# sumitsk/algp

Hardware: AMD Instinct MI355X
Metric: GP-fit+MI-score throughput (N train x M candidates) (higher is better)
Workload: dtype f64

## Files before the change

algp_amd/csrc/gemm.hip:

```cpp
#include "common.h"
#include <hip/hip_ext.h>
#include "mfma.h"
#include "gemm_sched.h"
#include <algorithm>
#include <type_traits>
#include <stdio.h>
#include <stdlib.h>

namespace algp {

template <typename T>
struct GemmArgs {
    const T* A;
    const T* B;
    const T* C;
    T* D;
    int64_t lda, ldb, ldc, ldd;
    int64_t sA, sB, sC, sD;
    int tiles_m, tiles_n, ktiles;
    T alpha, beta;
    int lower_only;
    int ktri;
    int kcut;
    const T* stat_w;
    T* stat_out;
    int64_t stat_ld;
    Sched sch;
    T* part;
};

template <typename T, int DP_, int FAM_ = 0>
struct GenGemmArgs : GemmArgs<T> {
    static constexpr int DP = DP_;
    static constexpr int FAM = FAM_;
    const T* rx;
    const T* cx;
    const int* rk;
    int64_t col0;
    int64_t ncols;
    int kernel;
    T os;
};
template <typename A>
struct gen_dp { static constexpr int value = 0; };
template <typename T, int DP, int FAM>
struct gen_dp<GenGemmArgs<T, DP, FAM>> { static constexpr int value = DP; };

typedef __attribute__((address_space(3))) void* lds_vp;
typedef const __attribute__((address_space(1))) void* glb_vp;

template <int CTRL>
__device__ __forceinline__ float dpp_row(float x) {
    return __int_as_float(__builtin_amdgcn_update_dpp(0, __float_as_int(x), CTRL, 0xf, 0xf, false));
}
template <int CTRL>
__device__ __forceinline__ double dpp_row(double x) {
    const int lo = __builtin_amdgcn_update_dpp(0, __double2loint(x), CTRL, 0xf, 0xf, false);
    const int hi = __builtin_amdgcn_update_dpp(0, __double2hiint(x), CTRL, 0xf, 0xf, false);
    return __hiloint2double(hi, lo);
}
template <typename T>
__device__ __forceinline__ T row16_sum(T x) {
    x += dpp_row<0x128>(x);
    x += dpp_row<0x124>(x);
    x += dpp_row<0x122>(x);
    x += dpp_row<0x121>(x);
    return x;
}

template <typename T>
struct VrGemmArgs : GemmArgs<T> {
    const int64_t* cidx;
    const int* ckind;
    int64_t M;
    union {
        int64_t ncol0;
        const int64_t* cpool;
    };
    const T* Xs;
    const T* Cp;
    int64_t n_pool;
    int DP, kernel;
    T os, noise;
    const T* tw;
};

template <typename T>
struct VrWGemmArgs : VrGemmArgs<T> {};
template <typename T>
struct VrxGemmArgs : VrGemmArgs<T> {};
template <typename T>
struct VrxWGemmArgs : VrxGemmArgs<T> {};

template <typename T>
__device__ __forceinline__ T vr_pool_cov(const VrGemmArgs<T>& g, int64_t prow, int64_t pcol, const T (&xrow)[MAXD], const T* xcol) {
    if (g.Cp) return g.Cp[prow * g.n_pool + pcol];
    T r2 = (T)0;
#pragma unroll
    for (int d = 0; d < MAXD; ++d) {
        const T df = xrow[d] - xcol[d];
        r2 += df * df;
    }
    T cv;
    if (g.kernel == ALGP_KERNEL_RBF) cv = g.os * kexp((T)-0.5 * r2);
    else if (g.kernel == ALGP_KERNEL_MATERN15) {
        const T rr = sqrt(r2) * (T)1.7320508075688772;
        cv = g.os * ((T)1 + rr) * kexp(-rr);
    } else cv = kval<T, 1>(g.kernel, g.os, r2);
    if (prow == pcol) cv += g.noise;
    return cv;
}

template <typename T, bool WEIGHTED, bool RECT, typename ACC>
__device__ __forceinline__ void vr_epilogue(const VrGemmArgs<T>& g, char* smem, const ACC (&acc)[4][4], int64_t m0, int64_t n0, int bn,
                                            int wr, int wc, int lane, int tid, const int64_t* cpool = nullptr) {
    using F = MF<T>;
    const int fr = lane & 15;
    T* red = reinterpret_cast<T*>(smem);
    T* xr = reinterpret_cast<T*>(smem + 2048);
    T* xc = reinterpret_cast<T*>(smem + 2048 + 8192);
    int64_t* pr = reinterpret_cast<int64_t*>(smem + 2048 + 16384);
    int64_t* pc = pr + 128;
    int* kr = reinterpret_cast<int*>(pc + 128);
    int* mc = kr + 128;
    T* wcol = reinterpret_cast<T*>(kr + 128);
    __syncthreads();
    {
        const int t = tid & 127;
        const bool is_col = tid >= 128;
        int64_t p;
        int ordinary;
        if (RECT && is_col) {
            const int64_t hp = cpool[n0 + t];
            ordinary = hp >= 0 ? 1 : 0;
            p = ordinary ? hp : 0;
        } else {
            const int64_t gi = (!RECT && is_col) ? g.ncol0 + n0 + t : m0 + t;
            const bool valid = gi < g.M;
            p = valid ? g.cidx[gi] : 0;
            ordinary = (valid && g.ckind[gi] < 0) ? 1 : 0;
        }
        (is_col ? pc : pr)[t] = p;
        if constexpr (WEIGHTED) {
            if (is_col) wcol[t] = ordinary ? g.tw[p] : (T)0;
            else kr[t] = ordinary;
        } else {
            (is_col ? mc : kr)[t] = ordinary;
        }
        if (!g.Cp) {
            T* x = (is_col ? xc : xr) + t * MAXD;
#pragma unroll
            for (int d = 0; d < MAXD; ++d) x[d] = d < g.DP ? g.Xs[p * g.DP + d] : (T)0;
        }
    }
    __syncthreads();
#pragma unroll
    for (int i = 0; i < 4; ++i)
#pragma unroll
        for (int r = 0; r < 4; ++r) {
            const int row = wr * 64 + i * 16 + F::row_of(lane, r);
            const int64_t prow = pr[row];
            const T kap = kr[row] ? (T)1 : (T)0;
            T xrow[MAXD];
#pragma unroll
            for (int d = 0; d < MAXD; ++d) xrow[d] = xr[row * MAXD + d];
            T s2 = (T)0;
            if constexpr (WEIGHTED) {
                T es[4], we[4];
#pragma unroll
                for (int j = 0; j < 4; ++j) {
                    const int col = wc * 64 + j * 16 + fr;
                    const int64_t pcol = pc[col];
                    const T cv = vr_pool_cov<T>(g, prow, pcol, xrow, xc + col * MAXD);
                    const T wgt = wcol[col];
                    const T e = kap * cv - acc[i][j][r];
                    es[j] = wgt != (T)0 ? e : (T)0;
                    we[j] = wgt * es[j];
                }
                s2 = kfma(we[0], es[0], we[1] * es[1]);
                s2 = kfma(we[2], es[2], s2);
                s2 = kfma(we[3], es[3], s2);
            } else {
#pragma unroll
                for (int j = 0; j < 4; ++j) {
                    const int col = wc * 64 + j * 16 + fr;
                    const int64_t pcol = pc[col];
                    const T cv = vr_pool_cov<T>(g, prow, pcol, xrow, xc + col * MAXD);
                    T e = kap * cv - acc[i][j][r];
                    e = mc[col] ? e : (T)0;
                    s2 += e * e;
                }
            }
            s2 = row16_sum<T>(s2);
            if (fr == 0) red[wc * 128 + row] = s2;
        }
    __syncthreads();
    if (tid < 128) g.stat_out[(int64_t)bn * g.stat_ld + m0 + tid] = red[tid] + red[128 + tid];
}

template <typename T>
struct PvrGemmArgs : VrGemmArgs<T> {
    const int64_t* uidx;
    int64_t U;
    T* E;
    int64_t lde;
};

template <typename T, typename ACC>
__device__ __forceinline__ void pvr_epilogue(const PvrGemmArgs<T>& g, char* smem, const ACC (&acc)[4][4], int64_t m0, int64_t n0, int wr,
                                             int wc, int lane, int tid) {
    using F = MF<T>;
    const int fr = lane & 15;
    T* xr = reinterpret_cast<T*>(smem);
    T* xc = reinterpret_cast<T*>(smem + 8192);
    int64_t* pr = reinterpret_cast<int64_t*>(smem + 16384);
    int64_t* pc = pr + 128;
    int* kr = reinterpret_cast<int*>(pc + 128);
    T* wcol = reinterpret_cast<T*>(kr + 128);
    __syncthreads();
    {
        const int t = tid & 127;
        const bool is_col = tid >= 128;
        const int64_t gi = is_col ? g.ncol0 + n0 + t : m0 + t;
        const bool valid = is_col ? gi < g.M : gi < g.U;
        const int64_t p = valid ? (is_col ? g.cidx[gi] : g.uidx[gi]) : 0;
        (is_col ? pc : pr)[t] = p;
        if (is_col) wcol[t] = (valid && g.ckind[gi] < 0) ? (g.tw ? sqrt(g.tw[p]) : (T)1) : (T)0;
        else kr[t] = valid ? 1 : 0;
        if (!g.Cp) {
            T* x = (is_col ? xc : xr) + t * MAXD;
#pragma unroll
            for (int d = 0; d < MAXD; ++d) x[d] = d < g.DP ? g.Xs[p * g.DP + d] : (T)0;
        }
    }
    __syncthreads();
#pragma unroll
    for (int i = 0; i < 4; ++i)
#pragma unroll
        for (int r = 0; r < 4; ++r) {
            const int row = wr * 64 + i * 16 + F::row_of(lane, r);
            const int64_t prow = pr[row];
            const bool rowon = kr[row] != 0;
            T xrow[MAXD];
#pragma unroll
            for (int d = 0; d < MAXD; ++d) xrow[d] = xr[row * MAXD + d];
            T* Er = g.E + (m0 + row) * g.lde + n0;
#pragma unroll
            for (int j = 0; j < 4; ++j) {
                const int col = wc * 64 + j * 16 + fr;
                const int64_t pcol = pc[col];
                const T cv = vr_pool_cov<T>(g, prow, pcol, xrow, xc + col * MAXD);
                const T sw = wcol[col];
                Er[col] = (rowon && sw != (T)0) ? sw * (cv - acc[i][j][r]) : (T)0;
            }
        }
}

#ifndef ALGP_GEMM_XOR_MASK
#define ALGP_GEMM_XOR_MASK 2
#endif
template <typename T, bool STATS = false, typename Args = GemmArgs<T>, bool SCHED = false>
__global__ __launch_bounds__(256, 2) void gemm_nt_kernel_dma4(Args g) {
    constexpr int GDP = gen_dp<Args>::value;
    constexpr bool GEN = GDP > 0;
    constexpr bool VR = std::is_base_of<VrGemmArgs<T>, Args>::value;
    static_assert(!(VR && STATS), "one epilogue per kernel");
    static_assert(!(VR && SCHED), "the scheduled form serves the sweep's products only");
    static_assert(!GEN || (SCHED && !STATS), "generated C tiles: the scheduled update product only");
    constexpr int NST = 4;
    using F = MF<T>;
    using acc_t = typename F::acc_t;
    using chunk_t = typename F::chunk_t;
    constexpr int EPC = F::EPC;
    constexpr int BK = 4 * EPC;

    constexpr int GEN_LDS = GEN ? 2 * 128 * GDP * (int)sizeof(T) + 128 * (int)sizeof(int) : 0;
    __shared__ __attribute__((aligned(1024))) char smem[NST * 16384 + (SCHED && STATS ? 4096 : 0) + GEN_LDS];

    const int nwg = gridDim.x;
    int bm, bn;
    int kskip = 0;
    int nkt;
    int slice = -1, nunits = 1, ui = 0;
    if constexpr (SCHED) {
        nunits = sched_count<!GEN>(g.sch, blockIdx.x);
        const SchedUnit u = sched_unit<!GEN>(g.sch, blockIdx.x, 0);
        bm = u.tile / g.tiles_n;
        bn = u.tile - bm * g.tiles_n;
        kskip = u.kb0 * (128 / BK);
        nkt = (u.kb1 - u.kb0) * (128 / BK);
        slice = u.slice;
    } else {
    if (g.ktri) {
        int local = blockIdx.x >> 3;
        bm = blockIdx.x & 7;
        while (bm < g.tiles_m && local > bm) { local -= bm + 1; bm += 8; }
        if (bm >= g.tiles_m) return;
        bn = local;
    } else {
        int sid;
        {
            const int id = blockIdx.x, xcd = id & 7, q = nwg >> 3, r = nwg & 7;
            sid = (xcd < r ? xcd * (q + 1) : r * (q + 1) + (xcd - r) * q) + (id >> 3);
        }
        if (g.lower_only) {
            bm = (int)((sqrt(8.0 * (double)sid + 1.0) - 1.0) * 0.5);
            while ((int64_t)(bm + 1) * (bm + 2) / 2 <= sid) ++bm;
            while ((int64_t)bm * (bm + 1) / 2 > sid) --bm;
            bn = sid - (int)((int64_t)bm * (bm + 1) / 2);
        } else {
            bm = sid / g.tiles_n;
            bn = sid - bm * g.tiles_n;
        }
    }
    kskip = g.ktri ? bm * (128 / BK) : 0;
    nkt = g.ktiles * 2 - kskip;
    if (g.kcut && (bn + 1) * (128 / BK) < nkt) nkt = (bn + 1) * (128 / BK);
    }
    const int tid = threadIdx.x, lane = tid & 63;
    const int wave = __builtin_amdgcn_readfirstlane(tid >> 6);
    const int wr = wave >> 1, wc = wave & 1;
    const int64_t bz = blockIdx.y;

    const int srow = lane >> 2;
    const int schunk = (lane & 3) ^ ((lane >> 4) & ALGP_GEMM_XOR_MASK);
    const T* Ag = g.A + bz * g.sA + ((int64_t)bm * 128 + 32 * wave + srow) * g.lda + schunk * EPC + (int64_t)kskip * BK;
    const T* Bg = g.B + bz * g.sB + ((int64_t)bn * 128 + 32 * wave + srow) * g.ldb + schunk * EPC + (int64_t)kskip * BK;
    auto stage = [&](int st, int kt) {
        char* As = smem + st * 16384 + wave * 2048;
        char* Bs = As + 8192;
#pragma unroll
        for (int i = 0; i < 2; ++i) {
            __builtin_amdgcn_global_load_lds((glb_vp)(Ag + (int64_t)(16 * i) * g.lda + (int64_t)kt * BK),
                                             (lds_vp)(As + i * 1024), 16, 0, 0);
            __builtin_amdgcn_global_load_lds((glb_vp)(Bg + (int64_t)(16 * i) * g.ldb + (int64_t)kt * BK),
                                             (lds_vp)(Bs + i * 1024), 16, 0, 0);
        }
    };

    const int fr = lane & 15, fg = lane >> 4;
    const int coff = ((fg ^ ((fr >> 2) & ALGP_GEMM_XOR_MASK)) << 4);
    const int aoff = (wr * 64 + fr) * 64 + coff;
    const int boff = (wc * 64 + fr) * 64 + coff;

    acc_t acc[4][4];
    typedef T gen_vec_t __attribute__((ext_vector_type(GEN ? GDP : 1)));
    gen_vec_t gx;
    int gk = -1;
    auto gen_load = [&](int ubm, int ubn) {
        if constexpr (GEN) {
            int t = tid & 127;
            asm volatile("" : "+v"(t));
            const int64_t row = (int64_t)ubm * 128 + t;
            const T* src = wave >= 2 ? g.cx + (g.col0 + (int64_t)ubn * 128 + t) * GDP : g.rx + row * GDP;
            gx = *reinterpret_cast<const gen_vec_t*>(src);
            gk = g.rk[row];
            asm volatile("" ::: "memory");
        }
    };
    gen_load(bm, bn);
#pragma unroll
    for (int t = 0; t < NST - 1; ++t)
        if (t < nkt) stage(t, t);

    auto fread = [&](int st, chunk_t (&a)[4], chunk_t (&b)[4]) {
        const char* As = smem + st * 16384;
        const char* Bs = As + 8192;
#pragma unroll
        for (int t = 0; t < 4; ++t) a[t] = *reinterpret_cast<const chunk_t*>(As + aoff + t * 1024);
#pragma unroll
        for (int t = 0; t < 4; ++t) b[t] = *reinterpret_cast<const chunk_t*>(Bs + boff + t * 1024);
    };
    auto fmac = [&](const chunk_t (&a)[4], const chunk_t (&b)[4]) {
#pragma unroll
        for (int j = 0; j < 4; ++j)
#pragma unroll
            for (int e = 0; e < EPC; ++e)
#pragma unroll
                for (int i = 0; i < 4; ++i) acc[i][j] = F::mfma(a[i][e], b[j][e], acc[i][j]);
    };
    auto arrive = [&](int younger) {
        if (younger >= 2) __builtin_amdgcn_s_waitcnt(0x0F78);
        else if (younger >= 1) __builtin_amdgcn_s_waitcnt(0x0F74);
        else __builtin_amdgcn_s_waitcnt(0x0F70);
        __builtin_amdgcn_s_barrier();
        asm volatile("" ::: "memory");
    };

    int st = 0;
    for (;;) {
#pragma unroll
    for (int i = 0; i < 4; ++i)
#pragma unroll
        for (int j = 0; j < 4; ++j)
#pragma unroll
            for (int r = 0; r < 4; ++r) acc[i][j][r] = (T)0;
    for (int kt = 0; kt < nkt; ++kt) {
        arrive(nkt - 1 - kt);
        chunk_t a[4], b[4];
        fread(st, a, b);
        if (kt + NST - 1 < nkt) stage(st == 0 ? NST - 1 : st - 1, kt + NST - 1);
        fmac(a, b);
        st = (st + 1 == NST) ? 0 : st + 1;
    }
    const int64_t m0 = (int64_t)bm * 128, n0 = (int64_t)bn * 128;
    const int cur_bn = bn, cur_slice = slice;
    if constexpr (GEN) {
        if (cur_slice < 0) {
            T* xr = reinterpret_cast<T*>(smem + NST * 16384);
            T* xc = xr + 128 * GDP;
            int* kr = reinterpret_cast<int*>(xc + 128 * GDP);
            int t = tid & 127;
            asm volatile("" : "+v"(t));
            *reinterpret_cast<gen_vec_t*>((wave >= 2 ? xc : xr) + t * GDP) = gx;
            if (wave < 2) kr[t] = gk;
        }
        asm volatile("" ::: "memory");
    }
    if constexpr (SCHED) {
        if (++ui < nunits) {
            const SchedUnit u = sched_unit<!GEN>(g.sch, blockIdx.x, ui);
            bm = u.tile / g.tiles_n;
            bn = u.tile - bm * g.tiles_n;
            nkt = (u.kb1 - u.kb0) * (128 / BK);
            slice = u.slice;
            gen_load(bm, bn);
            Ag = g.A + ((int64_t)bm * 128 + 32 * wave + srow) * g.lda + schunk * EPC + (int64_t)u.kb0 * 128;
            Bg = g.B + ((int64_t)bn * 128 + 32 * wave + srow) * g.ldb + schunk * EPC + (int64_t)u.kb0 * 128;
#pragma unroll
            for (int t = 0; t < NST - 1; ++t) stage((st + t) & (NST - 1), t);
        }
    }

    if constexpr (std::is_same<Args, PvrGemmArgs<T>>::value) {
        pvr_epilogue<T>(g, smem, acc, m0, n0, wr, wc, lane, tid);
        return;
    } else if constexpr (VR) {
        constexpr bool WEIGHTED = std::is_same<Args, VrWGemmArgs<T>>::value || std::is_same<Args, VrxWGemmArgs<T>>::value;
        if constexpr (std::is_base_of<VrxGemmArgs<T>, Args>::value)
            vr_epilogue<T, WEIGHTED, true>(g, smem, acc, m0, n0, (int)bz * g.tiles_n + cur_bn, wr, wc, lane, tid,
                                           reinterpret_cast<const int64_t*>(reinterpret_cast<const char*>(g.cpool) +
                                                                            bz * g.sB * (int64_t)sizeof(T)));
        else
            vr_epilogue<T, WEIGHTED, false>(g, smem, acc, m0, n0, cur_bn, wr, wc, lane, tid);
        return;
    }
    const T alpha = g.alpha, beta = g.beta;
    const T* Cb = g.C + bz * g.sC;
    T* Db = g.D + bz * g.sD;
    if (SCHED && !STATS && cur_slice >= 0) {
        T* P = g.part + (int64_t)cur_slice * (128 * 128);
#pragma unroll
        for (int i = 0; i < 4; ++i)
#pragma unroll
            for (int r = 0; r < 4; ++r) {
                const int row = wr * 64 + i * 16 + F::row_of(lane, r);
#pragma unroll
                for (int j = 0; j < 4; ++j) P[row * 128 + wc * 64 + j * 16 + fr] = alpha * acc[i][j][r];
            }
    } else if constexpr (GEN) {
        const T* xr = reinterpret_cast<const T*>(smem + NST * 16384);
        const T* xc = xr + 128 * GDP;
        const int* kr = reinterpret_cast<const int*>(xc + 128 * GDP);
        __builtin_amdgcn_s_waitcnt(0xC07F);
        __builtin_amdgcn_s_barrier();
        asm volatile("" ::: "memory");
        int ln = lane;
        asm volatile("" : "+v"(ln));
        const int gfr = ln & 15;
        T xcol[4][GDP];
#pragma unroll
        for (int j = 0; j < 4; ++j)
#pragma unroll
            for (int d = 0; d < GDP; ++d) xcol[j][d] = xc[(wc * 64 + j * 16 + gfr) * GDP + d];
        const int64_t gc = g.col0 + n0 + wc * 64 + gfr;
        const T os = g.os;
        const int64_t ncols = g.ncols;
        auto tile_out = [&](auto kform) {
#pragma unroll
            for (int i = 0; i < 4; ++i)
#pragma unroll
                for (int r = 0; r < 4; ++r) {
                    const int row = wr * 64 + i * 16 + F::row_of(ln, r);
                    T xrow[GDP];
#pragma unroll
                    for (int d = 0; d < GDP; ++d) xrow[d] = xr[row * GDP + d];
                    const int kind = kr[row];
                    T* Dr = Db + (m0 + row) * g.ldd + n0 + wc * 64 + gfr;
#pragma unroll
                    for (int j = 0; j < 4; ++j) {
                        const T cv = bt_entry<T, GDP>(decltype(kform)::value, os, xrow, xcol[j], kind, gc + 16 * j, ncols);
                        Dr[j * 16] = alpha * acc[i][j][r] + beta * cv;
                        if (j & 1) __builtin_amdgcn_sched_barrier(0);
                    }
                }
        };
        if constexpr (Args::FAM == 0) {
            if (g.kernel == ALGP_KERNEL_RBF) tile_out(std::integral_constant<int, ALGP_KERNEL_RBF>{});
            else tile_out(std::integral_constant<int, ALGP_KERNEL_MATERN15>{});
        } else {
            if (g.kernel == ALGP_KERNEL_MATERN05) tile_out(std::integral_constant<int, ALGP_KERNEL_MATERN05>{});
            else tile_out(std::integral_constant<int, ALGP_KERNEL_MATERN25>{});
        }
    } else if (beta != (T)0) {
#pragma unroll
        for (int i = 0; i < 4; ++i) {
            T cv[4][4];
#pragma unroll
            for (int r = 0; r < 4; ++r) {
                const int64_t gi = m0 + wr * 64 + i * 16 + F::row_of(lane, r);
#pragma unroll
                for (int j = 0; j < 4; ++j) cv[r][j] = Cb[gi * g.ldc + n0 + wc * 64 + j * 16 + fr];
            }
#pragma unroll
            for (int r = 0; r < 4; ++r) {
                const int64_t gi = m0 + wr * 64 + i * 16 + F::row_of(lane, r);
#pragma unroll
                for (int j = 0; j < 4; ++j)
                    Db[gi * g.ldd + n0 + wc * 64 + j * 16 + fr] = alpha * acc[i][j][r] + beta * cv[r][j];
            }
        }
    } else if (!STATS) {
#pragma unroll
        for (int i = 0; i < 4; ++i)
#pragma unroll
            for (int r = 0; r < 4; ++r) {
                const int64_t gi = m0 + wr * 64 + i * 16 + F::row_of(lane, r);
#pragma unroll
                for (int j = 0; j < 4; ++j) Db[gi * g.ldd + n0 + wc * 64 + j * 16 + fr] = alpha * acc[i][j][r];
            }
    } else {
        T wv[4];
#pragma unroll
        for (int j = 0; j < 4; ++j) wv[j] = g.stat_w[n0 + wc * 64 + j * 16 + fr];
        T* red = reinterpret_cast<T*>(smem + (SCHED ? NST * 16384 : 0));
        if constexpr (!SCHED) __syncthreads();
#pragma unroll
        for (int i = 0; i < 4; ++i)
#pragma unroll
            for (int r = 0; r < 4; ++r) {
                const int row = wr * 64 + i * 16 + F::row_of(lane, r);
                T s2 = (T)0, sw = (T)0;
#pragma unroll
                for (int j = 0; j < 4; ++j) {
                    const T d = alpha * acc[i][j][r];
                    Db[(m0 + row) * g.ldd + n0 + wc * 64 + j * 16 + fr] = d;
                    s2 += d * d;
                    sw += d * wv[j];
                }
                s2 = row16_sum<T>(s2);
                sw = row16_sum<T>(sw);
                if (fr == 0) {
                    red[(wc * 128 + row) * 2 + 0] = s2;
                    red[(wc * 128 + row) * 2 + 1] = sw;
                }
            }
        if constexpr (SCHED) {
            __builtin_amdgcn_s_waitcnt(0xC07F);
            __builtin_amdgcn_s_barrier();
            asm volatile("" ::: "memory");
        } else {
            __syncthreads();
        }
        const int row = tid >> 1, q = tid & 1;
        g.stat_out[(int64_t)(2 * cur_bn + q) * g.stat_ld + m0 + row] = red[row * 2 + q] + red[(128 + row) * 2 + q];
    }
    if constexpr (!SCHED) return;
    if (ui >= nunits) return;
    __builtin_amdgcn_s_waitcnt(0x0F70);
    }
}

constexpr int FIN_STRIPS = 16;
constexpr int FIN_BATCH = 8;
template <typename T>
struct Fin {
    static constexpr int EPV = 16 / (int)sizeof(T);
    static constexpr int RPW = 256 * EPV / 128;
    static constexpr int PPT = (128 / FIN_STRIPS) / RPW;
    static constexpr int RSTEP = RPW;
    typedef T V __attribute__((ext_vector_type(EPV)));
    static_assert(PPT >= 1 && PPT * RPW * FIN_STRIPS == 128, "a strip is whole passes of the workgroup");
};

template <typename T, int NB>
__device__ __forceinline__ void finish_add(const T* P, unsigned off, typename Fin<T>::V (&v)[Fin<T>::PPT]) {
#pragma clang fp contract(off)
    using F = Fin<T>;
    typename F::V p[NB][F::PPT];
#pragma unroll
    for (int b = 0; b < NB; ++b)
#pragma unroll
        for (int i = 0; i < F::PPT; ++i)
            p[b][i] = *reinterpret_cast<const typename F::V*>(P + b * (128 * 128) + (off + i * F::RSTEP * 128));
    __builtin_amdgcn_sched_barrier(0);
#pragma unroll
    for (int b = 0; b < NB; ++b)
#pragma unroll
        for (int i = 0; i < F::PPT; ++i) v[i] += p[b][i];
}

template <typename T>
__device__ __forceinline__ void finish_sum(const T* P, unsigned off, int S, typename Fin<T>::V (&v)[Fin<T>::PPT]) {
    int q = 0;
    for (; q + FIN_BATCH <= S; q += FIN_BATCH) finish_add<T, FIN_BATCH>(P + (int64_t)q * (128 * 128), off, v);
    static_assert(FIN_BATCH == 8, "the remainder below is 4 + 2 + 1");
    if ((S - q) & 4) { finish_add<T, 4>(P + (int64_t)q * (128 * 128), off, v); q += 4; }
    if ((S - q) & 2) { finish_add<T, 2>(P + (int64_t)q * (128 * 128), off, v); q += 2; }
    if ((S - q) & 1) finish_add<T, 1>(P + (int64_t)q * (128 * 128), off, v);
}

template <typename T>
__global__ __launch_bounds__(256) void gemm_finish_kernel(const T* part, int S, int tile0, int tiles_n, T beta, const T* C, int64_t ldc,
                                                          T* D, int64_t ldd) {
#pragma clang fp contract(off)
    using F = Fin<T>;
    using V = typename F::V;
    const int j = blockIdx.x / FIN_STRIPS, strip = blockIdx.x - j * FIN_STRIPS;
    const int tile = tile0 + j, bm = tile / tiles_n, bn = tile - bm * tiles_n;
    const int lrow = strip * (128 / FIN_STRIPS) + (int)threadIdx.x / (128 / F::EPV), lcol = ((int)threadIdx.x % (128 / F::EPV)) * F::EPV;
    const int64_t row = (int64_t)bm * 128 + lrow, col = (int64_t)bn * 128 + lcol;
    V v[F::PPT];
#pragma unroll
    for (int i = 0; i < F::PPT; ++i) v[i] = beta * *reinterpret_cast<const V*>(C + (row + i * F::RSTEP) * ldc + col);
    finish_sum<T>(part + (int64_t)j * S * (128 * 128), (unsigned)(lrow * 128 + lcol), S, v);
#pragma unroll
    for (int i = 0; i < F::PPT; ++i) *reinterpret_cast<V*>(D + (row + i * F::RSTEP) * ldd + col) = v[i];
}

template <typename T, int DP, int FAM>
__global__ __launch_bounds__(256) void gemm_finish_gen_kernel(const T* part, int S, int tile0, int tiles_n, T beta, const T* rx, const T* cx,
                                                              const int* rk, int64_t col0, int64_t ncols, int kernel, T os, T* D, int64_t ldd) {
#pragma clang fp contract(off)
    using F = Fin<T>;
    using V = typename F::V;
    const int j = blockIdx.x / FIN_STRIPS, strip = blockIdx.x - j * FIN_STRIPS;
    const int tile = tile0 + j, bm = tile / tiles_n, bn = tile - bm * tiles_n;
    const int lrow = strip * (128 / FIN_STRIPS) + (int)threadIdx.x / (128 / F::EPV), lcol = ((int)threadIdx.x % (128 / F::EPV)) * F::EPV;
    const int64_t row = (int64_t)bm * 128 + lrow, col = (int64_t)bn * 128 + lcol;
    T xcol[F::EPV][DP];
#pragma unroll
    for (int e = 0; e < F::EPV; ++e)
#pragma unroll
        for (int d = 0; d < DP; ++d) xcol[e][d] = cx[(col0 + col + e) * DP + d];
    T xrow[F::PPT][DP];
    int kind[F::PPT];
#pragma unroll
    for (int i = 0; i < F::PPT; ++i) {
#pragma unroll
        for (int d = 0; d < DP; ++d) xrow[i][d] = rx[(row + i * F::RSTEP) * DP + d];
        kind[i] = rk[row + i * F::RSTEP];
    }
    V v[F::PPT];
    auto c_term = [&](auto kform) {
#pragma clang fp contract(off)
#pragma unroll
        for (int i = 0; i < F::PPT; ++i) {
            V cv;
#pragma unroll
            for (int e = 0; e < F::EPV; ++e)
                cv[e] = bt_entry<T, DP>(decltype(kform)::value, os, xrow[i], xcol[e], kind[i], col0 + col + e, ncols);
            v[i] = beta * cv;
        }
    };
    if constexpr (FAM == 0) {
        if (kernel == ALGP_KERNEL_RBF) c_term(std::integral_constant<int, ALGP_KERNEL_RBF>{});
        else c_term(std::integral_constant<int, ALGP_KERNEL_MATERN15>{});
    } else {
        if (kernel == ALGP_KERNEL_MATERN05) c_term(std::integral_constant<int, ALGP_KERNEL_MATERN05>{});
        else c_term(std::integral_constant<int, ALGP_KERNEL_MATERN25>{});
    }
    finish_sum<T>(part + (int64_t)j * S * (128 * 128), (unsigned)(lrow * 128 + lcol), S, v);
#pragma unroll
    for (int i = 0; i < F::PPT; ++i) *reinterpret_cast<V*>(D + (row + i * F::RSTEP) * ldd + col) = v[i];
}

static void launch_log_line(int klass, int64_t m, int64_t n, int64_t k, int lower_only, int batch, int ktri, int es, int kcut) {
    static FILE* launch_log = getenv("ALGP_LAUNCH_LOG") ? fopen(getenv("ALGP_LAUNCH_LOG"), "w") : nullptr;
    if (!launch_log) return;
    fprintf(launch_log, "%d %lld %lld %lld %d %d %d %d %d\n", klass, (long long)m, (long long)n, (long long)k, lower_only, batch, ktri, es, kcut);
    fflush(launch_log);
}

template <typename T>
static int gemm_check(algp_ctx* c, const char* who, const GemmNt<T>& p, int64_t* tiles) {
    if (p.m % 128 || p.n % 128 || p.k % 128 || p.k <= 0 || p.A.ld % 4 || p.B.ld % 4 || p.A.stride % 4 || p.B.stride % 4)
        return fail(c, ALGP_ERR_BAD_ARG, std::string(who) + ": operands must be padded to multiples of 128");
    const int64_t tm = p.m / 128, tn = p.n / 128;
    *tiles = p.lower_only ? tm * (tm + 1) / 2 : tm * tn;
    if (*tiles > 0x7fffffff) return fail(c, ALGP_ERR_BAD_ARG, std::string(who) + ": grid too large");
    return ALGP_OK;
}

template <typename T>
static void gemm_fill(GemmArgs<T>& g, const GemmNt<T>& p) {
    const bool inplace = !p.C.p;
    g.A = p.A.p; g.B = p.B.p; g.C = inplace ? p.D.p : p.C.p; g.D = p.D.p;
    g.lda = p.A.ld; g.ldb = p.B.ld; g.ldc = inplace ? p.D.ld : p.C.ld; g.ldd = p.D.ld;
    g.sA = p.A.stride; g.sB = p.B.stride; g.sC = inplace ? p.D.stride : p.C.stride; g.sD = p.D.stride;
    g.tiles_m = (int)(p.m / 128);
    g.tiles_n = (int)(p.n / 128);
    g.ktiles = (int)(p.k / (8 * MF<T>::EPC));
    g.alpha = p.alpha; g.beta = p.beta;
    g.lower_only = p.lower_only;
    g.ktri = p.ktri;
    g.kcut = p.kcut;
    g.stat_w = p.stat_w;
    g.stat_out = p.stat_out;
    g.stat_ld = p.stat_ld;
    g.sch = Sched();
    g.part = nullptr;
}

struct Booking { double flops, bytes; };
template <typename T>
static Booking gemm_book(const GemmNt<T>& p, int64_t tiles, double tile_elems) {
    const double tm = (double)(p.m / 128), tn = (double)(p.n / 128);
    Booking b;
    b.flops = p.ktri ? 2.0 * 128.0 * 128.0 * 128.0 * tm * (tm + 1.0) * (tm + 2.0) / 6.0 * p.batch
              : p.kcut ? 2.0 * 128.0 * 128.0 * 128.0 * tm * tn * (tn + 1.0) / 2.0 * p.batch
                       : 2.0 * 128.0 * 128.0 * (double)p.k * (double)tiles * p.batch;
    b.bytes = sizeof(T) * p.batch * ((double)tiles * tile_elems + (double)p.k * 128.0 * (tm + tn));
    launch_log_line(p.klass, p.m, p.n, p.k, p.lower_only, p.batch, p.ktri, (int)sizeof(T), p.kcut);
    return b;
}

template <typename X>
struct as_is { typedef X type; };
template <typename... P>
static int dispatch(algp_ctx* c, int klass, double flops, double bytes, void (*kernel)(P...), dim3 grid, const typename as_is<P>::type&... args) {
    hipEvent_t ev_a, ev_b;
    if (prof_launch_events(c, klass, flops, bytes, &ev_a, &ev_b)) hipExtLaunchKernelGGL(kernel, grid, dim3(256), 0, c->cur, ev_a, ev_b, 0, args...);
    else hipLaunchKernelGGL(kernel, grid, dim3(256), 0, c->cur, args...);
    ALGP_HIP(hipGetLastError());
    return ALGP_OK;
}

template <typename T, typename Args, typename... Tail>
static int launch_scheduled(algp_ctx* c, const char* who, const GemmNt<T>& p, const Booking& bk, Args& g, void (*product)(Args),
                            void (*finish)(const T*, int, int, int, T, Tail...), bool c_loaded, const typename as_is<Tail>::type&... tail) {
    const int slots = 2 * c->cu_count;
    const bool split = p.beta != (T)0 && !p.stat_out && !p.kcut && c->gemm_part.p &&
                       c->gemm_part.cap >= sizeof(T) * 128 * 128 * (size_t)slots;
    g.sch = sched_make(slots, g.tiles_m, g.tiles_n, (int)(p.k / 128), p.kcut, split ? 1 : 0);
    g.part = (T*)c->gemm_part.p;
    if (g.sch.S >= 2 && (g.ldd % 4 || ((uintptr_t)g.D & 15) || (c_loaded && (g.ldc % 4 || ((uintptr_t)g.C & 15)))))
        return fail(c, ALGP_ERR_BAD_ARG, std::string(who) + ": the finish kernel moves its tiles in 16-byte pieces");
    ALGP_TRY(dispatch(c, p.klass, bk.flops, bk.bytes, product, dim3((unsigned)g.sch.G), g));
    if (g.sch.S >= 2)
        ALGP_TRY(dispatch(c, p.klass, 0.0, sizeof(T) * 128.0 * 128.0 * (double)g.sch.left * (g.sch.S + (c_loaded ? 2.0 : 1.0)), finish,
                          dim3((unsigned)(g.sch.left * FIN_STRIPS)), g.part, g.sch.S, g.sch.full, g.tiles_n, g.beta, tail...));
    return ALGP_OK;
}

template <typename T>
int gemm_nt(algp_ctx* c, const GemmNt<T>& p) {
    if (p.m <= 0 || p.n <= 0 || p.batch <= 0) return ALGP_OK;
    if (p.stat_out && (p.beta != (T)0 || p.batch != 1 || p.lower_only || p.ktri))
        return fail(c, ALGP_ERR_BAD_ARG, "gemm_nt: row statistics need beta = 0, no batch");
    if (p.kcut && (p.k != p.n || p.lower_only || p.ktri)) return fail(c, ALGP_ERR_BAD_ARG, "gemm_nt: kcut needs k == n");
    int64_t tiles;
    ALGP_TRY(gemm_check(c, "gemm_nt", p, &tiles));
    if (p.lower_only && p.m != p.n) return fail(c, ALGP_ERR_BAD_ARG, "gemm_nt: lower_only needs a square output");
    if (p.batch > 65535) return fail(c, ALGP_ERR_BAD_ARG, "gemm_nt: batch too large");
    if (p.ktri && (!p.lower_only || p.k != p.m)) return fail(c, ALGP_ERR_BAD_ARG, "gemm_nt: ktri needs a square lower-only product with k == m");
    GemmArgs<T> g;
    gemm_fill(g, p);
    const Booking bk = gemm_book(p, tiles, 128.0 * 128.0 * (p.beta != (T)0 ? 2.0 : 1.0));
    if (c->gemm_sched && c->cu_count > 0 && !p.lower_only && !p.ktri && p.batch == 1)
        return launch_scheduled(c, "gemm_nt", p, bk, g,
                                p.stat_out ? gemm_nt_kernel_dma4<T, true, GemmArgs<T>, true> : gemm_nt_kernel_dma4<T, false, GemmArgs<T>, true>,
                                gemm_finish_kernel<T>, true, g.C, g.ldc, g.D, g.ldd);
    int64_t gx = tiles;
    if (p.ktri) {
        int64_t most = 0;
        for (int x = 0; x < 8; ++x) {
            int64_t cnt = 0;
            for (int64_t r = x; r < g.tiles_m; r += 8) cnt += r + 1;
            most = std::max(most, cnt);
        }
        gx = 8 * most;
    }
    return dispatch(c, p.klass, bk.flops, bk.bytes, p.stat_out ? gemm_nt_kernel_dma4<T, true> : gemm_nt_kernel_dma4<T, false>,
                    dim3((unsigned)gx, (unsigned)p.batch), g);
}

bool rhs_gen_supported(int DP, bool pool_is_cov) { return DP == 2 && !pool_is_cov; }

template <typename T>
int gemm_nt_launch_gen(algp_ctx* c, int klass, int64_t m, int64_t n, int64_t k, T alpha, const T* A, int64_t lda, const T* B,
                       int64_t ldb, T beta, const RhsGen& gen, int64_t col0, T* D, int64_t ldd) {
    if (m <= 0 || n <= 0) return ALGP_OK;
    if (!c->gemm_sched || c->cu_count <= 0 || !rhs_gen_supported(gen.DP, false) || !gen.rx || !gen.cx || !gen.rk)
        return fail(c, ALGP_ERR_BAD_ARG, "gemm_nt_gen: the scheduled form with two gathered coordinates only");
    if (col0 < 0) return fail(c, ALGP_ERR_BAD_ARG, "gemm_nt_gen: operands must be padded to multiples of 128");
    const GemmNt<T> p = {.klass = klass, .m = m, .n = n, .k = k, .alpha = alpha, .beta = beta, .A = {A, lda}, .B = {B, ldb}, .D = {D, ldd}};
    int64_t tiles;
    ALGP_TRY(gemm_check(c, "gemm_nt_gen", p, &tiles));
    auto launch = [&](auto fam) {
        constexpr int FAM = decltype(fam)::value;
        GenGemmArgs<T, 2, FAM> g;
        gemm_fill(g, p);
        g.rx = (const T*)gen.rx; g.cx = (const T*)gen.cx; g.rk = gen.rk;
        g.col0 = col0; g.ncols = gen.ncols; g.kernel = gen.kernel; g.os = (T)gen.outputscale;
        return launch_scheduled(c, "gemm_nt_gen", p, gemm_book(p, tiles, 128.0 * 128.0), g,
                                gemm_nt_kernel_dma4<T, false, GenGemmArgs<T, 2, FAM>, true>, gemm_finish_gen_kernel<T, 2, FAM>, false, g.rx,
                                g.cx, g.rk, col0, g.ncols, g.kernel, g.os, D, ldd);
    };
    return kernel_family(gen.kernel) ? launch(std::integral_constant<int, 1>{}) : launch(std::integral_constant<int, 0>{});
}
template int gemm_nt_launch_gen<double>(algp_ctx*, int, int64_t, int64_t, int64_t, double, const double*, int64_t, const double*, int64_t,
                                        double, const RhsGen&, int64_t, double*, int64_t);
template int gemm_nt_launch_gen<float>(algp_ctx*, int, int64_t, int64_t, int64_t, float, const float*, int64_t, const float*, int64_t, float,
                                       const RhsGen&, int64_t, float*, int64_t);

template <typename T>
static void vr_fill(VrGemmArgs<T>& g, const KmatSrc& s, const int64_t* cidx, const int* ckind, int64_t M, int64_t ncol0, const T* tw) {
    g.cidx = cidx; g.ckind = ckind; g.M = M; g.ncol0 = ncol0; g.tw = tw;
    g.Xs = (const T*)s.Xs; g.Cp = (const T*)s.Cp; g.n_pool = s.n_pool; g.DP = s.DP; g.kernel = s.kernel;
    g.os = (T)s.outputscale; g.noise = (T)s.noise;
}

template <typename T>
int gemm_nt_launch_vr(algp_ctx* c, int klass, int64_t mpad, int64_t n, int64_t k, const T* Vt, int64_t ldv, int64_t ncol0,
                      const KmatSrc& s, const int64_t* cidx, const int* ckind, int64_t M, const T* tw, T* part, int64_t part_ld) {
    if (mpad <= 0 || n <= 0) return ALGP_OK;
    if (ncol0 % 128 || ncol0 + n > mpad || k > ldv || s.DP > MAXD)
        return fail(c, ALGP_ERR_BAD_ARG, "gemm_nt_vr: operands must be padded to multiples of 128");
    const GemmNt<T> p = {.klass = klass, .m = mpad, .n = n, .k = k, .A = {Vt, ldv}, .B = {Vt + ncol0 * ldv, ldv}, .stat_out = part, .stat_ld = part_ld};
    int64_t tiles;
    ALGP_TRY(gemm_check(c, "gemm_nt_vr", p, &tiles));
    VrGemmArgs<T> g;
    gemm_fill(g, p);
    vr_fill(g, s, cidx, ckind, M, ncol0, tw);
    const Booking bk = gemm_book(p, tiles, 128.0);
    if (!tw) return dispatch(c, klass, bk.flops, bk.bytes, gemm_nt_kernel_dma4<T, false, VrGemmArgs<T>>, dim3((unsigned)tiles), g);
    VrWGemmArgs<T> gw;
    static_cast<VrGemmArgs<T>&>(gw) = g;
    return dispatch(c, klass, bk.flops, bk.bytes, gemm_nt_kernel_dma4<T, false, VrWGemmArgs<T>>, dim3((unsigned)tiles), gw);
}
template int gemm_nt_launch_vr<double>(algp_ctx*, int, int64_t, int64_t, int64_t, const double*, int64_t, int64_t, const KmatSrc&,
                                       const int64_t*, const int*, int64_t, const double*, double*, int64_t);
template int gemm_nt_launch_vr<float>(algp_ctx*, int, int64_t, int64_t, int64_t, const float*, int64_t, int64_t, const KmatSrc&,
                                      const int64_t*, const int*, int64_t, const float*, float*, int64_t);

template <typename T>
int gemm_nt_launch_vrx(algp_ctx* c, int klass, int64_t mpad, int64_t n, int64_t k, const T* Vt, int64_t ldv, const T* B, int64_t ldb,
                       const int64_t* cpool, int nslices, int64_t slice_bytes, const KmatSrc& s, const int64_t* cidx, const int* ckind,
                       int64_t M, const T* tw, T* part, int64_t part_ld) {
    if (mpad <= 0 || n <= 0 || nslices <= 0) return ALGP_OK;
    if (k > ldv || k > ldb || s.DP > MAXD || !cpool || slice_bytes % 16 || ((uintptr_t)B & 15) || ((uintptr_t)cpool & 7) || nslices > 65535 ||
        (nslices > 1 && slice_bytes < (int64_t)sizeof(T) * n * ldb))
        return fail(c, ALGP_ERR_BAD_ARG, "gemm_nt_vrx: operands must be padded to multiples of 128, the slices 16-byte aligned");
    const GemmNt<T> p = {.klass = klass, .m = mpad, .n = n, .k = k, .A = {Vt, ldv}, .B = {B, ldb, slice_bytes / (int64_t)sizeof(T)},
                         .batch = nslices, .stat_out = part, .stat_ld = part_ld};
    int64_t tiles;
    ALGP_TRY(gemm_check(c, "gemm_nt_vrx", p, &tiles));
    VrxGemmArgs<T> g;
    gemm_fill(g, p);
    vr_fill(g, s, cidx, ckind, M, 0, tw);
    g.cpool = cpool;
    const Booking bk = gemm_book(p, tiles, 128.0);
    const dim3 grid((unsigned)tiles, (unsigned)nslices);
    if (!tw) return dispatch(c, klass, bk.flops, bk.bytes, gemm_nt_kernel_dma4<T, false, VrxGemmArgs<T>>, grid, g);
    VrxWGemmArgs<T> gw;
    static_cast<VrGemmArgs<T>&>(gw) = g;
    return dispatch(c, klass, bk.flops, bk.bytes, gemm_nt_kernel_dma4<T, false, VrxWGemmArgs<T>>, grid, gw);
}
template int gemm_nt_launch_vrx<double>(algp_ctx*, int, int64_t, int64_t, int64_t, const double*, int64_t, const double*, int64_t,
                                        const int64_t*, int, int64_t, const KmatSrc&, const int64_t*, const int*, int64_t, const double*,
                                        double*, int64_t);
template int gemm_nt_launch_vrx<float>(algp_ctx*, int, int64_t, int64_t, int64_t, const float*, int64_t, const float*, int64_t,
                                       const int64_t*, int, int64_t, const KmatSrc&, const int64_t*, const int*, int64_t, const float*,
                                       float*, int64_t);

template <typename T>
int gemm_nt_launch_pvr(algp_ctx* c, int klass, int64_t upad, int64_t n, int64_t k, const T* R, int64_t ldr, const T* Vt, int64_t ldv,
                       int64_t ncol0, const KmatSrc& s, const int64_t* uidx, int64_t U, const int64_t* cidx, const int* ckind, int64_t M,
                       const T* tw, T* E, int64_t lde) {
    if (upad <= 0 || n <= 0) return ALGP_OK;
    if (ncol0 % 128 || ncol0 + n > (M + 127) / 128 * 128 || k > ldv || k > ldr || U > upad || lde < n || s.DP > MAXD)
        return fail(c, ALGP_ERR_BAD_ARG, "gemm_nt_pvr: operands must be padded to multiples of 128");
    const GemmNt<T> p = {.klass = klass, .m = upad, .n = n, .k = k, .A = {R, ldr}, .B = {Vt + ncol0 * ldv, ldv}};
    int64_t tiles;
    ALGP_TRY(gemm_check(c, "gemm_nt_pvr", p, &tiles));
    PvrGemmArgs<T> g;
    gemm_fill(g, p);
    vr_fill(g, s, cidx, ckind, M, ncol0, tw);
    g.uidx = uidx; g.U = U; g.E = E; g.lde = lde;
    const Booking bk = gemm_book(p, tiles, 128.0 * 128.0);
    return dispatch(c, klass, bk.flops, bk.bytes, gemm_nt_kernel_dma4<T, false, PvrGemmArgs<T>>, dim3((unsigned)tiles), g);
}
template int gemm_nt_launch_pvr<double>(algp_ctx*, int, int64_t, int64_t, int64_t, const double*, int64_t, const double*, int64_t, int64_t,
                                        const KmatSrc&, const int64_t*, int64_t, const int64_t*, const int*, int64_t, const double*, double*,
                                        int64_t);
template int gemm_nt_launch_pvr<float>(algp_ctx*, int, int64_t, int64_t, int64_t, const float*, int64_t, const float*, int64_t, int64_t,
                                       const KmatSrc&, const int64_t*, int64_t, const int64_t*, const int*, int64_t, const float*, float*,
                                       int64_t);

template <typename T>
int gemm_nt_launch(algp_ctx* c, int klass, int64_t m, int64_t n, int64_t k, T alpha, const T* A,
                   int64_t lda, const T* B, int64_t ldb, T beta, const T* C, int64_t ldc, T* D,
                   int64_t ldd, int lower_only) {
    return gemm_nt<T>(c, {.klass = klass, .m = m, .n = n, .k = k, .alpha = alpha, .beta = beta, .A = {A, lda}, .B = {B, ldb}, .C = {C, ldc},
                          .D = {D, ldd}, .lower_only = lower_only});
}
template <typename T>
int gemm_nt_launch_stats(algp_ctx* c, int klass, int64_t m, int64_t k, T alpha, const T* A, int64_t lda, const T* B, int64_t ldb,
                         T* D, int64_t ldd, const T* w, T* stat_out, int64_t stat_ld) {
    return gemm_nt<T>(c, {.klass = klass, .m = m, .n = 128, .k = k, .alpha = alpha, .A = {A, lda}, .B = {B, ldb}, .D = {D, ldd},
                          .stat_w = w, .stat_out = stat_out, .stat_ld = stat_ld});
}
template <typename T>
int gemm_nt_launch_tri(algp_ctx* c, int klass, int64_t m, int64_t n, const T* A, int64_t lda, const T* B, int64_t ldb, T* D,
                       int64_t ldd, const T* w, T* stat_out, int64_t stat_ld) {
    return gemm_nt<T>(c, {.klass = klass, .m = m, .n = n, .k = n, .A = {A, lda}, .B = {B, ldb}, .D = {D, ldd}, .kcut = 1,
                          .stat_w = stat_out ? w : nullptr, .stat_out = stat_out, .stat_ld = stat_ld});
}
template int gemm_nt_launch_tri<double>(algp_ctx*, int, int64_t, int64_t, const double*, int64_t, const double*, int64_t, double*,
                                        int64_t, const double*, double*, int64_t);
template int gemm_nt_launch_tri<float>(algp_ctx*, int, int64_t, int64_t, const float*, int64_t, const float*, int64_t, float*, int64_t,
                                       const float*, float*, int64_t);
template int gemm_nt_launch_stats<double>(algp_ctx*, int, int64_t, int64_t, double, const double*, int64_t, const double*, int64_t,
                                          double*, int64_t, const double*, double*, int64_t);
template int gemm_nt_launch_stats<float>(algp_ctx*, int, int64_t, int64_t, float, const float*, int64_t, const float*, int64_t, float*,
                                         int64_t, const float*, float*, int64_t);

template int gemm_nt_launch<double>(algp_ctx*, int, int64_t, int64_t, int64_t, double, const double*, int64_t,
                                    const double*, int64_t, double, const double*, int64_t, double*, int64_t, int);
template int gemm_nt_launch<float>(algp_ctx*, int, int64_t, int64_t, int64_t, float, const float*, int64_t,
                                   const float*, int64_t, float, const float*, int64_t, float*, int64_t, int);
template int gemm_nt<double>(algp_ctx*, const GemmNt<double>&);
template int gemm_nt<float>(algp_ctx*, const GemmNt<float>&);

template <typename T>
__global__ void mfma_probe_kernel(int* mismatches) {
    using F = MF<T>;
    const int lane = threadIdx.x & 63;
    const int i = lane & 15, kk = lane >> 4;
    const T a = (T)(i * 4 + kk + 1);
    const T b = (T)((kk + 1) * 17 + i * 3);
    typename F::acc_t acc;
    for (int r = 0; r < 4; ++r) acc[r] = (T)0;
    acc = F::mfma(a, b, acc);
    int bad = 0;
    for (int r = 0; r < 4; ++r) {
        const int row = F::row_of(lane, r), col = lane & 15;
        double want = 0;
        for (int k = 0; k < 4; ++k) want += (double)(row * 4 + k + 1) * (double)((k + 1) * 17 + col * 3);
        if ((double)acc[r] != want) ++bad;
    }
    if (bad) atomicAdd(mismatches, bad);
}

template <typename T>
int test_mfma_launch(algp_ctx* c, int* mismatches_dev) {
    hipLaunchKernelGGL(mfma_probe_kernel<T>, dim3(1), dim3(64), 0, c->cur, mismatches_dev);
    ALGP_HIP(hipGetLastError());
    return ALGP_OK;
}
template int test_mfma_launch<double>(algp_ctx*, int*);
template int test_mfma_launch<float>(algp_ctx*, int*);


template <typename T>
__global__ void fill_random_kernel(T* p, int64_t n, unsigned seed) {
    const int64_t i = (int64_t)blockIdx.x * blockDim.x + threadIdx.x;
    if (i >= n) return;
    unsigned x = (unsigned)(i * 2654435761u) ^ seed;
    x ^= x >> 16; x *= 0x7feb352du; x ^= x >> 15; x *= 0x846ca68bu; x ^= x >> 16;
    p[i] = (T)((int)(x & 0xffff) - 32768) * (T)(1.0 / 32768.0);
}

template <typename T>
int bench_gemm(algp_ctx* c, int64_t m, int64_t n, int64_t k, int lower_only, int beta_one, int reps,
               double* ms_out, bool gen_c) {
    DevBuf a, b, cc;
    int rc = ensure(c, a, sizeof(T) * m * k);
    if (rc == ALGP_OK) rc = ensure(c, b, sizeof(T) * n * k);
    if (rc == ALGP_OK) rc = ensure(c, cc, sizeof(T) * m * n);
    if (rc != ALGP_OK) { hipFree(a.p); hipFree(b.p); hipFree(cc.p); return rc; }
    hipLaunchKernelGGL(fill_random_kernel<T>, dim3((unsigned)((m * k + 255) / 256)), dim3(256), 0, c->cur, (T*)a.p, m * k, 1u);
    hipLaunchKernelGGL(fill_random_kernel<T>, dim3((unsigned)((n * k + 255) / 256)), dim3(256), 0, c->cur, (T*)b.p, n * k, 2u);
    hipLaunchKernelGGL(fill_random_kernel<T>, dim3((unsigned)((m * n + 255) / 256)), dim3(256), 0, c->cur, (T*)cc.p, m * n, 3u);
    hipEvent_t e0, e1;
    hipEventCreate(&e0);
    hipEventCreate(&e1);
    const T beta = beta_one ? (T)1 : (T)0;
    DevBuf grx, gcx, grk;
    RhsGen gen;
    if (gen_c) {
        rc = ensure(c, grx, sizeof(T) * m * 2);
        if (rc == ALGP_OK) rc = ensure(c, gcx, sizeof(T) * n * 2);
        if (rc == ALGP_OK) rc = ensure(c, grk, sizeof(int) * m);
        if (rc == ALGP_OK) {
            hipLaunchKernelGGL(fill_random_kernel<T>, dim3((unsigned)((m * 2 + 255) / 256)), dim3(256), 0, c->cur, (T*)grx.p, m * 2, 4u);
            hipLaunchKernelGGL(fill_random_kernel<T>, dim3((unsigned)((n * 2 + 255) / 256)), dim3(256), 0, c->cur, (T*)gcx.p, n * 2, 5u);
            hipMemsetAsync(grk.p, 0xff, sizeof(int) * m, c->cur);
            gen.rx = grx.p; gen.cx = gcx.p; gen.rk = (const int*)grk.p;
            gen.ncols = n; gen.DP = 2; gen.kernel = ALGP_KERNEL_RBF; gen.outputscale = 1.0;
        }
    }
    auto one = [&]() {
        if (gen_c) return gemm_nt_launch_gen<T>(c, ALGP_PROF_GEMM_OTHER, m, n, k, (T)-1, (const T*)a.p, k, (const T*)b.p, k, beta, gen, 0, (T*)cc.p, n);
        return gemm_nt_launch<T>(c, ALGP_PROF_GEMM_OTHER, m, n, k, (T)-1, (const T*)a.p, k, (const T*)b.p, k, beta, (const T*)cc.p, n,
                                 (T*)cc.p, n, lower_only);
    };
    const bool sched = !lower_only && c->cu_count > 0 && env_switch("ALGP_TRSM_SCHED", true) &&
                       ensure(c, c->gemm_part, sizeof(T) * 128 * 128 * 2 * (size_t)c->cu_count) == ALGP_OK;
    c->gemm_sched = sched;
    for (int w = 0; w < 2 && rc == ALGP_OK; ++w) rc = one();
    hipEventRecord(e0, c->cur);
    for (int r = 0; r < reps && rc == ALGP_OK; ++r) rc = one();
    hipEventRecord(e1, c->cur);
    c->gemm_sched = false;
    hipEventSynchronize(e1);
    float ms = 0;
    hipEventElapsedTime(&ms, e0, e1);
    *ms_out = ms / (reps > 0 ? reps : 1);
    hipEventDestroy(e0);
    hipEventDestroy(e1);
    hipFree(a.p); hipFree(b.p); hipFree(cc.p); hipFree(grx.p); hipFree(gcx.p); hipFree(grk.p);
    c->dev_bytes -= (int64_t)(a.cap + b.cap + cc.cap + grx.cap + gcx.cap + grk.cap);
    return rc;
}
template int bench_gemm<double>(algp_ctx*, int64_t, int64_t, int64_t, int, int, int, double*, bool);
template int bench_gemm<float>(algp_ctx*, int64_t, int64_t, int64_t, int, int, int, double*, bool);

}
```

Before: 650,400.

## Add triangular-B GEMM form that skips zero blocks and folds row stats in-register

Adds a TRI template variant of the DMA GEMM kernel for the kcut (triangular B, k==n) products. Each wave now owns 32 rows across all 128 columns, and in the final diagonal 128-wide k-block it skips MFMAs and LDS reads for column groups that are structurally zero. The row-statistics epilogue becomes a per-wave reduction with no LDS staging or barrier, and the stats launch now routes through kcut. The 2x8 accumulator layout changes register pressure and B-fragment reuse compared with the 4x4 layout.

```diff
diff --git a/algp_amd/csrc/gemm.hip b/algp_amd/csrc/gemm.hip
--- a/algp_amd/csrc/gemm.hip
+++ b/algp_amd/csrc/gemm.hip
@@ -259,12 +259,14 @@
 #ifndef ALGP_GEMM_XOR_MASK
 #define ALGP_GEMM_XOR_MASK 2
 #endif
-template <typename T, bool STATS = false, typename Args = GemmArgs<T>, bool SCHED = false>
+template <typename T, bool STATS = false, typename Args = GemmArgs<T>, bool SCHED = false, bool TRI = false>
 __global__ __launch_bounds__(256, 2) void gemm_nt_kernel_dma4(Args g) {
     constexpr int GDP = gen_dp<Args>::value;
     constexpr bool GEN = GDP > 0;
     constexpr bool VR = std::is_base_of<VrGemmArgs<T>, Args>::value;
     static_assert(!(VR && STATS), "one epilogue per kernel");
+    static_assert(!TRI || (!VR && !GEN), "the triangular form serves the sweep's block-inverse products only");
+    static_assert(!STATS || TRI, "row statistics ride on the triangular form");
     static_assert(!(VR && SCHED), "the scheduled form serves the sweep's products only");
     static_assert(!GEN || (SCHED && !STATS), "generated C tiles: the scheduled update product only");
     constexpr int NST = 4;
@@ -275,7 +277,7 @@
     constexpr int BK = 4 * EPC;
 
     constexpr int GEN_LDS = GEN ? 2 * 128 * GDP * (int)sizeof(T) + 128 * (int)sizeof(int) : 0;
-    __shared__ __attribute__((aligned(1024))) char smem[NST * 16384 + (SCHED && STATS ? 4096 : 0) + GEN_LDS];
+    __shared__ __attribute__((aligned(1024))) char smem[NST * 16384 + GEN_LDS];
 
     const int nwg = gridDim.x;
     int bm, bn;
@@ -340,10 +342,11 @@
 
     const int fr = lane & 15, fg = lane >> 4;
     const int coff = ((fg ^ ((fr >> 2) & ALGP_GEMM_XOR_MASK)) << 4);
-    const int aoff = (wr * 64 + fr) * 64 + coff;
-    const int boff = (wc * 64 + fr) * 64 + coff;
-
-    acc_t acc[4][4];
+    const int aoff = ((TRI ? wave * 32 : wr * 64) + fr) * 64 + coff;
+    const int boff = ((TRI ? 0 : wc * 64) + fr) * 64 + coff;
+
+    constexpr int AI = TRI ? 2 : 4, AJ = TRI ? 8 : 4;
+    acc_t acc[AI][AJ];
     typedef T gen_vec_t __attribute__((ext_vector_type(GEN ? GDP : 1)));
     gen_vec_t gx;
     int gk = -1;
@@ -363,7 +366,7 @@
     for (int t = 0; t < NST - 1; ++t)
         if (t < nkt) stage(t, t);
 
-    auto fread = [&](int st, chunk_t (&a)[4], chunk_t (&b)[4]) {
+    auto fread = [&](int st, auto& a, auto& b) {
         const char* As = smem + st * 16384;
         const char* Bs = As + 8192;
 #pragma unroll
@@ -371,7 +374,7 @@
 #pragma unroll
         for (int t = 0; t < 4; ++t) b[t] = *reinterpret_cast<const chunk_t*>(Bs + boff + t * 1024);
     };
-    auto fmac = [&](const chunk_t (&a)[4], const chunk_t (&b)[4]) {
+    auto fmac = [&](const auto& a, const auto& b) {
 #pragma unroll
         for (int j = 0; j < 4; ++j)
 #pragma unroll
@@ -387,14 +390,53 @@
         asm volatile("" ::: "memory");
     };
 
+    auto tri_tile = [&](int st, int next_kt, int g0) {
+        const char* As = smem + st * 16384;
+        const char* Bs = As + 8192;
+        chunk_t a[2];
+#pragma unroll
+        for (int t = 0; t < 2; ++t) a[t] = *reinterpret_cast<const chunk_t*>(As + aoff + t * 1024);
+#pragma unroll
+        for (int h = 0; h < 2; ++h) {
+            chunk_t b[4];
+#pragma unroll
+            for (int t = 0; t < 4; ++t)
+                if (4 * h + t >= g0) b[t] = *reinterpret_cast<const chunk_t*>(Bs + boff + (4 * h + t) * 1024);
+            if (h == 0 && next_kt >= 0) stage(st == 0 ? NST - 1 : st - 1, next_kt);
+#pragma unroll
+            for (int t = 0; t < 4; ++t)
+                if (4 * h + t >= g0) {
+#pragma unroll
+                    for (int e = 0; e < EPC; ++e)
+#pragma unroll
+                        for (int i = 0; i < 2; ++i) acc[i][4 * h + t] = F::mfma(a[i][e], b[t][e], acc[i][4 * h + t]);
+                }
+        }
+    };
+
     int st = 0;
     for (;;) {
 #pragma unroll
-    for (int i = 0; i < 4; ++i)
-#pragma unroll
-        for (int j = 0; j < 4; ++j)
+    for (int i = 0; i < AI; ++i)
+#pragma unroll
+        for (int j = 0; j < AJ; ++j)
 #pragma unroll
             for (int r = 0; r < 4; ++r) acc[i][j][r] = (T)0;
+    if constexpr (TRI) {
+        constexpr int NKD = 128 / BK;
+        const int nk1 = nkt - NKD;
+        for (int kt = 0; kt < nk1; ++kt) {
+            arrive(2);
+            tri_tile(st, kt + NST - 1, 0);
+            st = (st + 1 == NST) ? 0 : st + 1;
+        }
+#pragma unroll
+        for (int kd = 0; kd < NKD; ++kd) {
+            arrive(NKD - 1 - kd);
+            tri_tile(st, kd + NST - 1 < NKD ? nk1 + kd + NST - 1 : -1, kd * BK / 16);
+            st = (st + 1 == NST) ? 0 : st + 1;
+        }
+    } else {
     for (int kt = 0; kt < nkt; ++kt) {
         arrive(nkt - 1 - kt);
         chunk_t a[4], b[4];
@@ -402,6 +444,7 @@
         if (kt + NST - 1 < nkt) stage(st == 0 ? NST - 1 : st - 1, kt + NST - 1);
         fmac(a, b);
         st = (st + 1 == NST) ? 0 : st + 1;
+    }
     }
     const int64_t m0 = (int64_t)bm * 128, n0 = (int64_t)bn * 128;
     const int cur_bn = bn, cur_slice = slice;
@@ -445,10 +488,49 @@
             vr_epilogue<T, WEIGHTED, false>(g, smem, acc, m0, n0, cur_bn, wr, wc, lane, tid);
         return;
     }
+    if constexpr (TRI) {
+        const T alpha = g.alpha;
+        T* Db = g.D + bz * g.sD;
+        T wv[8];
+        if constexpr (STATS) {
+#pragma unroll
+            for (int j = 0; j < 8; ++j) wv[j] = g.stat_w[n0 + j * 16 + fr];
+        }
+#pragma unroll
+        for (int i = 0; i < 2; ++i)
+#pragma unroll
+            for (int r = 0; r < 4; ++r) {
+                const int64_t gi = m0 + wave * 32 + i * 16 + F::row_of(lane, r);
+                T s2[2], sw[2];
+#pragma unroll
+                for (int h = 0; h < 2; ++h) {
+                    s2[h] = (T)0, sw[h] = (T)0;
+#pragma unroll
+                    for (int j = 4 * h; j < 4 * h + 4; ++j) {
+                        const T d = alpha * acc[i][j][r];
+                        Db[gi * g.ldd + n0 + j * 16 + fr] = d;
+                        if constexpr (STATS) {
+                            s2[h] += d * d;
+                            sw[h] += d * wv[j];
+                        }
+                    }
+                    if constexpr (STATS) {
+                        s2[h] = row16_sum<T>(s2[h]);
+                        sw[h] = row16_sum<T>(sw[h]);
+                    }
+                }
+                if constexpr (STATS) {
+                    if (fr == 0) {
+                        g.stat_out[(int64_t)(2 * cur_bn + 0) * g.stat_ld + gi] = s2[0] + s2[1];
+                        g.stat_out[(int64_t)(2 * cur_bn + 1) * g.stat_ld + gi] = sw[0] + sw[1];
+                    }
+                }
+            }
+    } else {
     const T alpha = g.alpha, beta = g.beta;
     const T* Cb = g.C + bz * g.sC;
     T* Db = g.D + bz * g.sD;
-    if (SCHED && !STATS && cur_slice >= 0) {
+    if (SCHED && cur_slice >= 0) {
         T* P = g.part + (int64_t)cur_slice * (128 * 128);
 #pragma unroll
         for (int i = 0; i < 4; ++i)
@@ -520,7 +602,7 @@
                     Db[gi * g.ldd + n0 + wc * 64 + j * 16 + fr] = alpha * acc[i][j][r] + beta * cv[r][j];
             }
         }
-    } else if (!STATS) {
+    } else {
 #pragma unroll
         for (int i = 0; i < 4; ++i)
 #pragma unroll
@@ -529,41 +611,7 @@
 #pragma unroll
                 for (int j = 0; j < 4; ++j) Db[gi * g.ldd + n0 + wc * 64 + j * 16 + fr] = alpha * acc[i][j][r];
             }
-    } else {
-        T wv[4];
-#pragma unroll
-        for (int j = 0; j < 4; ++j) wv[j] = g.stat_w[n0 + wc * 64 + j * 16 + fr];
-        T* red = reinterpret_cast<T*>(smem + (SCHED ? NST * 16384 : 0));
-        if constexpr (!SCHED) __syncthreads();
-#pragma unroll
-        for (int i = 0; i < 4; ++i)
-#pragma unroll
-            for (int r = 0; r < 4; ++r) {
-                const int row = wr * 64 + i * 16 + F::row_of(lane, r);
-                T s2 = (T)0, sw = (T)0;
-#pragma unroll
-                for (int j = 0; j < 4; ++j) {
-                    const T d = alpha * acc[i][j][r];
-                    Db[(m0 + row) * g.ldd + n0 + wc * 64 + j * 16 + fr] = d;
-                    s2 += d * d;
-                    sw += d * wv[j];
-                }
-                s2 = row16_sum<T>(s2);
-                sw = row16_sum<T>(sw);
-                if (fr == 0) {
-                    red[(wc * 128 + row) * 2 + 0] = s2;
-                    red[(wc * 128 + row) * 2 + 1] = sw;
-                }
-            }
-        if constexpr (SCHED) {
-            __builtin_amdgcn_s_waitcnt(0xC07F);
-            __builtin_amdgcn_s_barrier();
-            asm volatile("" ::: "memory");
-        } else {
-            __syncthreads();
-        }
-        const int row = tid >> 1, q = tid & 1;
-        g.stat_out[(int64_t)(2 * cur_bn + q) * g.stat_ld + m0 + row] = red[row * 2 + q] + red[(128 + row) * 2 + q];
+    }
     }
     if constexpr (!SCHED) return;
     if (ui >= nunits) return;
@@ -756,9 +804,9 @@
 template <typename T>
 int gemm_nt(algp_ctx* c, const GemmNt<T>& p) {
     if (p.m <= 0 || p.n <= 0 || p.batch <= 0) return ALGP_OK;
-    if (p.stat_out && (p.beta != (T)0 || p.batch != 1 || p.lower_only || p.ktri))
-        return fail(c, ALGP_ERR_BAD_ARG, "gemm_nt: row statistics need beta = 0, no batch");
-    if (p.kcut && (p.k != p.n || p.lower_only || p.ktri)) return fail(c, ALGP_ERR_BAD_ARG, "gemm_nt: kcut needs k == n");
+    if (p.stat_out && (!p.kcut || p.batch != 1)) return fail(c, ALGP_ERR_BAD_ARG, "gemm_nt: row statistics need kcut, no batch");
+    if (p.kcut && (p.k != p.n || p.lower_only || p.ktri || p.beta != (T)0))
+        return fail(c, ALGP_ERR_BAD_ARG, "gemm_nt: kcut needs k == n, beta = 0");
     int64_t tiles;
     ALGP_TRY(gemm_check(c, "gemm_nt", p, &tiles));
     if (p.lower_only && p.m != p.n) return fail(c, ALGP_ERR_BAD_ARG, "gemm_nt: lower_only needs a square output");
@@ -767,10 +815,13 @@
     GemmArgs<T> g;
     gemm_fill(g, p);
     const Booking bk = gemm_book(p, tiles, 128.0 * 128.0 * (p.beta != (T)0 ? 2.0 : 1.0));
+    auto form = [&](auto sched) -> void (*)(GemmArgs<T>) {
+        constexpr bool S = decltype(sched)::value;
+        if (!p.kcut) return gemm_nt_kernel_dma4<T, false, GemmArgs<T>, S>;
+        return p.stat_out ? gemm_nt_kernel_dma4<T, true, GemmArgs<T>, S, true> : gemm_nt_kernel_dma4<T, false, GemmArgs<T>, S, true>;
+    };
     if (c->gemm_sched && c->cu_count > 0 && !p.lower_only && !p.ktri && p.batch == 1)
-        return launch_scheduled(c, "gemm_nt", p, bk, g,
-                                p.stat_out ? gemm_nt_kernel_dma4<T, true, GemmArgs<T>, true> : gemm_nt_kernel_dma4<T, false, GemmArgs<T>, true>,
-                                gemm_finish_kernel<T>, true, g.C, g.ldc, g.D, g.ldd);
+        return launch_scheduled(c, "gemm_nt", p, bk, g, form(std::true_type{}), gemm_finish_kernel<T>, true, g.C, g.ldc, g.D, g.ldd);
     int64_t gx = tiles;
     if (p.ktri) {
         int64_t most = 0;
@@ -781,8 +832,7 @@
         }
         gx = 8 * most;
     }
-    return dispatch(c, p.klass, bk.flops, bk.bytes, p.stat_out ? gemm_nt_kernel_dma4<T, true> : gemm_nt_kernel_dma4<T, false>,
-                    dim3((unsigned)gx, (unsigned)p.batch), g);
+    return dispatch(c, p.klass, bk.flops, bk.bytes, form(std::false_type{}), dim3((unsigned)gx, (unsigned)p.batch), g);
 }
 
 bool rhs_gen_supported(int DP, bool pool_is_cov) { return DP == 2 && !pool_is_cov; }
@@ -909,7 +959,7 @@
 int gemm_nt_launch_stats(algp_ctx* c, int klass, int64_t m, int64_t k, T alpha, const T* A, int64_t lda, const T* B, int64_t ldb,
                          T* D, int64_t ldd, const T* w, T* stat_out, int64_t stat_ld) {
     return gemm_nt<T>(c, {.klass = klass, .m = m, .n = 128, .k = k, .alpha = alpha, .A = {A, lda}, .B = {B, ldb}, .D = {D, ldd},
-                          .stat_w = w, .stat_out = stat_out, .stat_ld = stat_ld});
+                          .kcut = 1, .stat_w = w, .stat_out = stat_out, .stat_ld = stat_ld});
 }
 template <typename T>
 int gemm_nt_launch_tri(algp_ctx* c, int klass, int64_t m, int64_t n, const T* A, int64_t lda, const T* B, int64_t ldb, T* D,
```

Result: no change. 656,000, median of 6 (+0.9%).
